# UBCMOCCA/mocca_envs

Measured on AMD Instinct MI355X. Metric: env-steps/sec, Walker3DCustomEnv-v0 @ 4096 envs, 1/2/4/8 MI355X, higher is better.
Workload: dtype f32; 1 GPU; Walker3DCustomEnv-v0, 4096 envs/GPU, flat ground, U(-1,1) action tape, auto-reset; max_rows=48, max_contacts=12, envs_per_gpu=4096, parallelism=independent env shards x1, no collective, preroll_steps=6096

## Files before the change

mocca_envs_amd/csrc/mocca_device.h:

```cpp
#pragma once

#include <hip/hip_runtime.h>
#include <stdint.h>

#include "mocca_model.h"
#include "mocca_philox.h"
#include "topo_walker3d.h"
#include "topo_cassie.h"
#include "topo_walker2d.h"
#include "topo_crab2d.h"
#include "topo_laikago.h"

#define DI __device__ __forceinline__

#ifndef MOCCA_NS
#define MOCCA_NS mocca
#endif
#ifndef MOCCA_MAXR
#define MOCCA_MAXR 48
#endif
#ifndef MOCCA_COMPACT
#define MOCCA_COMPACT 0
#endif

// ... 166 lines not shown
  unsigned long long* pace_acc;
  float* ep_ret;
  float* ep_masks;
  float* ep_bad;
  void* ep_rec;
  float* ep_totals;
  uint32_t ep_serial;
  float* robot_state;
  const float* base_value;
  int32_t* hf_field;
  int hf_stride, hf_n_fields, hf_redraw;
};
constexpr int ROBOT_STATE_STRIDE = 64;

DI void read_kernargs(StepArgs& la) {
  auto p = __builtin_amdgcn_kernarg_segment_ptr();
  asm volatile("" : "+s"(p));
  __builtin_memcpy(&la, p, sizeof(StepArgs));
}
template <bool LATE>
DI void late_args(StepArgs& la) {
  if constexpr (LATE) read_kernargs(la);
}
template <class T, int TASK, bool INJECT>
#ifdef MOCCA_NO_TRIM_7
constexpr bool LATE_ARGS = false;
#else
constexpr bool LATE_ARGS = INJECT || MAXR > 48 || !__is_base_of(TopoWalker3D, T) || (!COMPACT && TASK == MOCCA_TASK_WALKER3D_CUSTOM);
#endif

DI void wsync() {
  __builtin_amdgcn_fence(__ATOMIC_RELEASE, "wavefront");
  __builtin_amdgcn_wave_barrier();
  __builtin_amdgcn_fence(__ATOMIC_ACQUIRE, "wavefront");
}
DI float dot3(const float* a, const float* b) { return a[0] * b[0] + a[1] * b[1] + a[2] * b[2]; }
DI void cross3(const float* a, const float* b, float* o) {
  float x = a[1] * b[2] - a[2] * b[1], y = a[2] * b[0] - a[0] * b[2], z = a[0] * b[1] - a[1] * b[0];
  o[0] = x; o[1] = y; o[2] = z;
}
DI float dot6(const float* a, const float* b) {
  return a[0] * b[0] + a[1] * b[1] + a[2] * b[2] + a[3] * b[3] + a[4] * b[4] + a[5] * b[5];
}
DI void matvec3(const float* R, const float* x, float* o) {
  float a = R[0] * x[0] + R[1] * x[1] + R[2] * x[2];
  float b = R[3] * x[0] + R[4] * x[1] + R[5] * x[2];
// ... 489 lines not shown
        for (int k = 0; k < j; ++k) t -= own[k] * Afac[sym(j, k)];
        Afac[sym(j, j)] = readlane(rsq(t), j);
        own[j] = t * Afac[sym(j, j)];
#pragma unroll
        for (int i = j + 1; i < 6; ++i) Afac[sym(i, j)] = readlane(own[j], i);
      }
      chol6_solve(Afac, pA, a0);
    } else {
      float IA[21], pA[6];
#pragma unroll
      for (int i = 0; i < 6; ++i) {
        const float4 lo = *reinterpret_cast<const float4*>(L + L_B0 + 8 * i), hi = *reinterpret_cast<const float4*>(L + L_B0 + 8 * i + 4);
        const float rr_[6] = {lo.x, lo.y, lo.z, lo.w, hi.x, hi.y};
#pragma unroll
        for (int j = i; j < 6; ++j) IA[sym(i, j)] = rr_[j];
        pA[i] = hi.z;
      }
      float Ai[21];
      chol6_factor(IA, Ai);
      chol6_solve(Ai, pA, a0);
#pragma unroll
      for (int i = 0; i < 21; ++i) Afac[i] = unif(Ai[i]);
    }
#pragma unroll
    for (int i = 0; i < 6; ++i) abase[i] = -a0[i];
  }
  STAMP(11);
  {
    const int b = lane < T::NB ? lane : 0;
    float a[6], qdd = 0;
#pragma unroll
    for (int i = 0; i < 6; ++i) a[i] = abase[i];
#pragma unroll
    for (int k = 0; k < T::MAXD; ++k) {
      const int j = (int)((ppk >> (5 * k)) & 31ull);
      if (j != 0) {
        float U[6], S[6];
#pragma unroll
        for (int i = 0; i < 6; ++i) { a[i] += L[L_SV + SVS * j + SV_C + i]; U[i] = L[L_SV + SVS * j + SV_V + i]; S[i] = L[L_SV + SVS * j + i]; }
        qdd = L[L_SV + SVS * j + SV_UU] - dot6(U, a);
#pragma unroll
        for (int i = 0; i < 6; ++i) a[i] += S[i] * qdd;
      }
    }
    const float dt = M->dt;
    if (lane >= 1 && lane < T::NB) L[L_NU + 5 + b] = L[L_QD + b] + dt * qdd;
    if (lane == 0) {
      float om[3] = {L[L_BASE + 10], L[L_BASE + 11], L[L_BASE + 12]}, vl[3] = {L[L_BASE + 7], L[L_BASE + 8], L[L_BASE + 9]}, wxv[3];
      cross3(om, vl, wxv);
#pragma unroll
      for (int i = 0; i < 3; ++i) {
        L[L_NU + i] = om[i] + dt * a[i];
        L[L_NU + 3 + i] = vl[i] + dt * (a[3 + i] + wxv[i]);
      }
    }
    wsync();
  }
  STAMP(12);
}

DI void plane_space(const float* n, float* t1, float* t2) {
  if (fabsf(n[2]) > 0.70710678f) {
    const float a = n[1] * n[1] + n[2] * n[2], k = rsq(a);
    t1[0] = 0; t1[1] = -n[2] * k; t1[2] = n[1] * k;
    t2[0] = a * k; t2[1] = -n[0] * t1[2]; t2[2] = n[0] * t1[1];
  } else {
    const float a = n[0] * n[0] + n[1] * n[1], k = rsq(a);
    t1[0] = -n[1] * k; t1[1] = n[0] * k; t1[2] = 0;
    t2[0] = -n[2] * t1[1]; t2[1] = n[2] * t1[0]; t2[2] = a * k;
// ... 1808 lines not shown
```

mocca_envs_amd/csrc/mocca_kernels.h:

```cpp
#pragma once
#include <hip/hip_runtime.h>

#include "mocca.h"
#include "mocca_device.h"

namespace MOCCA_NS {

#ifndef MOCCA_WAVES_PER_EU
#define MOCCA_WAVES_PER_EU 4
#endif

DI void flush_obs(const float* L, float* dst, int lane, int obs_dim) {
#pragma unroll 1
  for (int k = lane; k < obs_dim; k += 64) dst[k] = L[L_OBS + k];
}
DI void keep_terminal_obs(const StepArgs& a, const float* L, int env, int lane) {
  wsync();
  if (a.final_obs) flush_obs(L, a.final_obs + (size_t)env * a.obs_dim, lane, a.obs_dim);
  wsync();
}

template <class T>
DI void keep_robot_state(const StepArgs& a, const float* L, int env, int lane) {
  static_assert(ROBOT_OBS<T> <= 64 && ROBOT_OBS<T> <= ROBOT_STATE_STRIDE, "one store per lane");
// ... 203 lines not shown
  cassie_observe(M, L, lane, cs, t.initz, jv, phase, obs);
  return {rew, 0};
}

template <class T, int TASK, bool INJECT = false>
__global__ __launch_bounds__(64, MOCCA_WAVES_PER_EU) void mocca_step_kernel(StepArgs a) {
  __shared__ float L[L_TOTAL];
  const int lane = threadIdx.x;
  if ((int)blockIdx.x >= a.n_envs) return;
  const int env = a.order ? uni(a.order[blockIdx.x]) : (int)blockIdx.x;
  ModelP M = (ModelP)a.model;
  float* st = a.dyn + (size_t)env * DYN_STRIDE;
  uint32_t* tk = a.task + (size_t)env * MOCCA_TASK_WORDS;
  float* ter = TASK == MOCCA_TASK_WALKER3D_STEPPER ? a.terrain + (size_t)env * TERRAIN_STRIDE : nullptr;
  float* obs_out = a.obs + (size_t)env * a.obs_dim;
  float* obs = L + L_OBS;
  int32_t* dbg = a.dbg ? a.dbg + (size_t)env * MOCCA_DEBUG_WORDS : nullptr;

  const bool warm_ld = INJECT || uni(__float_as_int(M->warmstart)) != 0, warm_st = warm_ld || a.persist_warm != 0;
  if (dbg && lane == 0) { dbg[16] = 0; dbg[17] = 0; dbg[18] = 0; }
  load_dyn(st, L, lane, T::NJ, T::NSLOT, warm_ld);
  pace_start(a, L, lane, INJECT ? 0 : a.pace);
  if (lane == 0) L[L_KEEPWARM] = __int_as_float((warm_st ? 1 : 0) | ((a.prio & PRIO_DELASSUS_VALU) ? 2 : 0));
  const unsigned long long ppk = T::path_packed(lane < T::NB ? lane : 0);
  ContactFlags fl = {0, 0, 0, 0, 0, 0, 0, 0, 0};
  int cover = 0;
  constexpr bool LATE = LATE_ARGS<T, TASK, INJECT>;
  StepArgs late, late_reset;
  const StepArgs& al = LATE ? late : a;
  if constexpr (TASK == MOCCA_TASK_CASSIE) {
    const int no = M->n_ordered, nctl = M->n_ctrl, mode = M->cassie_mode;
    float target = 0.0f;
    if (lane < nctl) {
      float base = M->ctrl_base[lane];
      if (mode != MOCCA_CASSIE_PLAIN) {
        const int f0 = traj_frame(a, M, (int)tk[MOCCA_TW_ISTEP]);
        base = (lane < nctl - 2 && M->residual_control) ? a.traj[(size_t)f0 * MOCCA_TRAJ_STRIDE + M->ctrl_oidx[lane]] : 0.0f;
      }
      target = base + (lane < nctl - 2 ? a.act[(size_t)env * (nctl - 2) + lane] : 0.0f);
    }
    if (lane < no) {
      L[L_JVEL + lane] = __uint_as_float(tk[MOCCA_TW_JVEL + lane]);
      L[L_Q0 + lane] = L[L_Q + M->ordered_body[lane]];
    }
    if (lane < MOCCA_MAX_BODIES) L[L_TAU + lane] = 0.0f;
    if (lane == 0) { L[L_Q] = 0.0f; L[L_QD] = 0.0f; }
    wsync();
// ... 212 lines not shown
```

mocca_envs_amd/csrc/topo_cassie.h:

```cpp
#pragma once
__device__ static const signed char kPathCassie[19][7] = {
  {-1, -1, -1, -1, -1, -1, -1},
  {1, -1, -1, -1, -1, -1, -1},
  {1, 2, -1, -1, -1, -1, -1},
  {1, 2, 3, -1, -1, -1, -1},
  {1, 2, 3, 4, -1, -1, -1},
  {1, 2, 3, 4, 5, -1, -1},
  {1, 2, 3, 4, 5, 6, -1},
  {1, 2, 3, 4, 5, 6, 7},
  {1, 2, 3, 8, -1, -1, -1},
  {1, 2, 3, 8, 9, -1, -1},
  {10, -1, -1, -1, -1, -1, -1},
  {10, 11, -1, -1, -1, -1, -1},
  {10, 11, 12, -1, -1, -1, -1},
  {10, 11, 12, 13, -1, -1, -1},
  {10, 11, 12, 13, 14, -1, -1},
  {10, 11, 12, 13, 14, 15, -1},
  {10, 11, 12, 13, 14, 15, 16},
  {10, 11, 12, 17, -1, -1, -1},
  {10, 11, 12, 17, 18, -1, -1},
};
__device__ static const signed char kChildCassie[19][2] = {
  {10, 1},
  {2, -1},
// ... 6 lines not shown
  {9, -1},
  {-1, -1},
  {11, -1},
  {12, -1},
  {17, 13},
  {14, -1},
  {15, -1},
  {16, -1},
  {-1, -1},
  {18, -1},
  {-1, -1},
};
__device__ static const signed char kLevelCassie[8][4] = {
  {-1, -1, -1, -1},
  {1, 10, -1, -1},
  {2, 11, -1, -1},
  {3, 12, -1, -1},
  {4, 13, 8, 17},
  {5, 14, 9, 18},
  {6, 15, -1, -1},
  {7, 16, -1, -1},
};
__device__ static const unsigned long long kPathPkCassie[19] = {0x0ull, 0x1ull, 0x41ull, 0xc41ull, 0x20c41ull, 0x520c41ull, 0xc520c41ull, 0x1cc520c41ull, 0x40c41ull, 0x940c41ull, 0xaull, 0x16aull, 0x316aull, 0x6b16aull, 0xe6b16aull, 0x1ee6b16aull, 0x41ee6b16aull, 0x8b16aull, 0x128b16aull};
struct TopoCassie {
  static constexpr int NB = 19;
  static constexpr int NJ = 18;
  static constexpr int ND = 24;
  static constexpr int MAXD = 7;
  static constexpr int MAXCH = 2;
  static constexpr int MAXW = 4;
  static constexpr int NG = 24;
  static constexpr int NSLOT = 24;
  static constexpr int NPAIR = 0;
  static constexpr int NCLOS = 2;
  static constexpr int NFEET = 2;
  static constexpr int parent(int b) { constexpr int t[19] = {-1, 0, 1, 2, 3, 4, 5, 6, 3, 8, 0, 10, 11, 12, 13, 14, 15, 12, 17}; return t[b]; }
  static constexpr int depth(int b) { constexpr int t[19] = {0, 1, 2, 3, 4, 5, 6, 7, 4, 5, 1, 2, 3, 4, 5, 6, 7, 4, 5}; return t[b]; }
  static constexpr unsigned anc_mask(int b) { constexpr unsigned t[19] = {0x0u, 0x2u, 0x6u, 0xeu, 0x1eu, 0x3eu, 0x7eu, 0xfeu, 0x10eu, 0x30eu, 0x400u, 0xc00u, 0x1c00u, 0x3c00u, 0x7c00u, 0xfc00u, 0x1fc00u, 0x21c00u, 0x61c00u}; return t[b]; }
  static __device__ __forceinline__ int path(int b, int k) { return kPathCassie[b][k]; }
  static __device__ __forceinline__ int child(int b, int k) { return kChildCassie[b][k]; }
  static __device__ __forceinline__ int level(int d, int s) { return kLevelCassie[d][s]; }
  static constexpr int clevel(int d, int s) { constexpr int t[8][4] = {{-1, -1, -1, -1}, {1, 10, -1, -1}, {2, 11, -1, -1}, {3, 12, -1, -1}, {4, 13, 8, 17}, {5, 14, 9, 18}, {6, 15, -1, -1}, {7, 16, -1, -1}}; return t[d][s]; }
  static constexpr bool massless(int b) { constexpr bool t[19] = {false, false, false, false, false, false, false, false, true, false, false, false, false, false, false, false, false, true, false}; return b >= 0 && t[b]; }
  static constexpr int ccarry(int b) { constexpr int t[19] = {-1, 2, 3, 4, 5, 6, 7, -1, 9, -1, 11, 12, 13, 14, 15, 16, -1, 18, -1}; return b < 0 ? -1 : t[b]; }
  static constexpr int cchild(int b, int k) { constexpr int t[19][2] = {{10, 1}, {2, -1}, {3, -1}, {8, 4}, {5, -1}, {6, -1}, {7, -1}, {-1, -1}, {9, -1}, {-1, -1}, {11, -1}, {12, -1}, {17, 13}, {14, -1}, {15, -1}, {16, -1}, {-1, -1}, {18, -1}, {-1, -1}}; return b < 0 ? -1 : t[b][k]; }
  static __device__ __forceinline__ unsigned long long path_packed(int b) { return kPathPkCassie[b]; }
};
```

mocca_envs_amd/csrc/topo_crab2d.h:

```cpp
#pragma once
__device__ static const signed char kPathCrab2D[7][3] = {
  {-1, -1, -1},
  {1, -1, -1},
  {1, 2, -1},
  {1, 2, 3},
  {4, -1, -1},
  {4, 5, -1},
  {4, 5, 6},
};
__device__ static const signed char kChildCrab2D[7][2] = {
  {4, 1},
  {2, -1},
  {3, -1},
  {-1, -1},
  {5, -1},
  {6, -1},
  {-1, -1},
};
__device__ static const signed char kLevelCrab2D[4][4] = {
  {-1, -1, -1, -1},
  {1, 4, -1, -1},
  {2, 5, -1, -1},
  {3, 6, -1, -1},
};
__device__ static const unsigned long long kPathPkCrab2D[7] = {0x0ull, 0x1ull, 0x41ull, 0xc41ull, 0x4ull, 0xa4ull, 0x18a4ull};
struct TopoCrab2D {
  static constexpr int NB = 7;
  static constexpr int NJ = 6;
  static constexpr int ND = 12;
  static constexpr int MAXD = 3;
  static constexpr int MAXCH = 2;
  static constexpr int MAXW = 4;
  static constexpr int NG = 7;
  static constexpr int NSLOT = 14;
  static constexpr int NPAIR = 9;
  static constexpr int NCLOS = 0;
  static constexpr int NFEET = 2;
  static constexpr int parent(int b) { constexpr int t[7] = {-1, 0, 1, 2, 0, 4, 5}; return t[b]; }
  static constexpr int depth(int b) { constexpr int t[7] = {0, 1, 2, 3, 1, 2, 3}; return t[b]; }
  static constexpr unsigned anc_mask(int b) { constexpr unsigned t[7] = {0x0u, 0x2u, 0x6u, 0xeu, 0x10u, 0x30u, 0x70u}; return t[b]; }
  static __device__ __forceinline__ int path(int b, int k) { return kPathCrab2D[b][k]; }
  static __device__ __forceinline__ int child(int b, int k) { return kChildCrab2D[b][k]; }
  static __device__ __forceinline__ int level(int d, int s) { return kLevelCrab2D[d][s]; }
  static constexpr int clevel(int d, int s) { constexpr int t[4][4] = {{-1, -1, -1, -1}, {1, 4, -1, -1}, {2, 5, -1, -1}, {3, 6, -1, -1}}; return t[d][s]; }
  static constexpr bool massless(int b) { constexpr bool t[7] = {false, false, false, false, false, false, false}; return b >= 0 && t[b]; }
  static constexpr int ccarry(int b) { constexpr int t[7] = {-1, 2, 3, -1, 5, 6, -1}; return b < 0 ? -1 : t[b]; }
  static constexpr int cchild(int b, int k) { constexpr int t[7][2] = {{4, 1}, {2, -1}, {3, -1}, {-1, -1}, {5, -1}, {6, -1}, {-1, -1}}; return b < 0 ? -1 : t[b][k]; }
  static __device__ __forceinline__ unsigned long long path_packed(int b) { return kPathPkCrab2D[b]; }
};
```

mocca_envs_amd/csrc/topo_laikago.h:

```cpp
#pragma once
__device__ static const signed char kPathLaikago[13][3] = {
  {-1, -1, -1},
  {1, -1, -1},
  {1, 2, -1},
  {1, 2, 3},
  {4, -1, -1},
  {4, 5, -1},
  {4, 5, 6},
  {7, -1, -1},
  {7, 8, -1},
  {7, 8, 9},
  {10, -1, -1},
  {10, 11, -1},
  {10, 11, 12},
};
__device__ static const signed char kChildLaikago[13][4] = {
  {10, 7, 4, 1},
  {2, -1, -1, -1},
  {3, -1, -1, -1},
  {-1, -1, -1, -1},
  {5, -1, -1, -1},
  {6, -1, -1, -1},
  {-1, -1, -1, -1},
  {8, -1, -1, -1},
  {9, -1, -1, -1},
  {-1, -1, -1, -1},
  {11, -1, -1, -1},
  {12, -1, -1, -1},
  {-1, -1, -1, -1},
};
__device__ static const signed char kLevelLaikago[4][4] = {
  {-1, -1, -1, -1},
  {1, 4, 7, 10},
  {2, 5, 8, 11},
  {3, 6, 9, 12},
};
__device__ static const unsigned long long kPathPkLaikago[13] = {0x0ull, 0x1ull, 0x41ull, 0xc41ull, 0x4ull, 0xa4ull, 0x18a4ull, 0x7ull, 0x107ull, 0x2507ull, 0xaull, 0x16aull, 0x316aull};
struct TopoLaikago {
  static constexpr int NB = 13;
  static constexpr int NJ = 12;
  static constexpr int ND = 18;
  static constexpr int MAXD = 3;
  static constexpr int MAXCH = 4;
  static constexpr int MAXW = 4;
  static constexpr int NG = 32;
  static constexpr int NSLOT = 32;
  static constexpr int NPAIR = 0;
  static constexpr int NCLOS = 0;
  static constexpr int NFEET = 4;
  static constexpr int parent(int b) { constexpr int t[13] = {-1, 0, 1, 2, 0, 4, 5, 0, 7, 8, 0, 10, 11}; return t[b]; }
  static constexpr int depth(int b) { constexpr int t[13] = {0, 1, 2, 3, 1, 2, 3, 1, 2, 3, 1, 2, 3}; return t[b]; }
  static constexpr unsigned anc_mask(int b) { constexpr unsigned t[13] = {0x0u, 0x2u, 0x6u, 0xeu, 0x10u, 0x30u, 0x70u, 0x80u, 0x180u, 0x380u, 0x400u, 0xc00u, 0x1c00u}; return t[b]; }
  static __device__ __forceinline__ int path(int b, int k) { return kPathLaikago[b][k]; }
  static __device__ __forceinline__ int child(int b, int k) { return kChildLaikago[b][k]; }
  static __device__ __forceinline__ int level(int d, int s) { return kLevelLaikago[d][s]; }
  static constexpr int clevel(int d, int s) { constexpr int t[4][4] = {{-1, -1, -1, -1}, {1, 4, 7, 10}, {2, 5, 8, 11}, {3, 6, 9, 12}}; return t[d][s]; }
  static constexpr bool massless(int b) { constexpr bool t[13] = {false, false, false, false, false, false, false, false, false, false, false, false, false}; return b >= 0 && t[b]; }
  static constexpr int ccarry(int b) { constexpr int t[13] = {-1, 2, 3, -1, 5, 6, -1, 8, 9, -1, 11, 12, -1}; return b < 0 ? -1 : t[b]; }
  static constexpr int cchild(int b, int k) { constexpr int t[13][4] = {{10, 7, 4, 1}, {2, -1, -1, -1}, {3, -1, -1, -1}, {-1, -1, -1, -1}, {5, -1, -1, -1}, {6, -1, -1, -1}, {-1, -1, -1, -1}, {8, -1, -1, -1}, {9, -1, -1, -1}, {-1, -1, -1, -1}, {11, -1, -1, -1}, {12, -1, -1, -1}, {-1, -1, -1, -1}}; return b < 0 ? -1 : t[b][k]; }
  static __device__ __forceinline__ unsigned long long path_packed(int b) { return kPathPkLaikago[b]; }
};
```

mocca_envs_amd/csrc/topo_walker2d.h:

```cpp
#pragma once
__device__ static const signed char kPathWalker2D[8][3] = {
  {-1, -1, -1},
  {1, -1, -1},
  {2, -1, -1},
  {2, 3, -1},
  {2, 3, 4},
  {5, -1, -1},
  {5, 6, -1},
  {5, 6, 7},
};
__device__ static const signed char kChildWalker2D[8][3] = {
  {5, 2, 1},
  {-1, -1, -1},
  {3, -1, -1},
  {4, -1, -1},
  {-1, -1, -1},
  {6, -1, -1},
  {7, -1, -1},
  {-1, -1, -1},
};
__device__ static const signed char kLevelWalker2D[4][4] = {
  {-1, -1, -1, -1},
  {2, 5, 1, -1},
  {3, 6, -1, -1},
  {4, 7, -1, -1},
};
__device__ static const unsigned long long kPathPkWalker2D[8] = {0x0ull, 0x1ull, 0x2ull, 0x62ull, 0x1062ull, 0x5ull, 0xc5ull, 0x1cc5ull};
struct TopoWalker2D {
  static constexpr int NB = 8;
  static constexpr int NJ = 7;
  static constexpr int ND = 13;
  static constexpr int MAXD = 3;
  static constexpr int MAXCH = 3;
  static constexpr int MAXW = 4;
  static constexpr int NG = 8;
  static constexpr int NSLOT = 15;
  static constexpr int NPAIR = 0;
  static constexpr int NCLOS = 0;
  static constexpr int NFEET = 2;
  static constexpr int parent(int b) { constexpr int t[8] = {-1, 0, 0, 2, 3, 0, 5, 6}; return t[b]; }
  static constexpr int depth(int b) { constexpr int t[8] = {0, 1, 1, 2, 3, 1, 2, 3}; return t[b]; }
  static constexpr unsigned anc_mask(int b) { constexpr unsigned t[8] = {0x0u, 0x2u, 0x4u, 0xcu, 0x1cu, 0x20u, 0x60u, 0xe0u}; return t[b]; }
  static __device__ __forceinline__ int path(int b, int k) { return kPathWalker2D[b][k]; }
  static __device__ __forceinline__ int child(int b, int k) { return kChildWalker2D[b][k]; }
  static __device__ __forceinline__ int level(int d, int s) { return kLevelWalker2D[d][s]; }
  static constexpr int clevel(int d, int s) { constexpr int t[4][4] = {{-1, -1, -1, -1}, {2, 5, 1, -1}, {3, 6, -1, -1}, {4, 7, -1, -1}}; return t[d][s]; }
  static constexpr bool massless(int b) { constexpr bool t[8] = {false, false, false, false, false, false, false, false}; return b >= 0 && t[b]; }
  static constexpr int ccarry(int b) { constexpr int t[8] = {-1, -1, 3, 4, -1, 6, 7, -1}; return b < 0 ? -1 : t[b]; }
  static constexpr int cchild(int b, int k) { constexpr int t[8][3] = {{5, 2, 1}, {-1, -1, -1}, {3, -1, -1}, {4, -1, -1}, {-1, -1, -1}, {6, -1, -1}, {7, -1, -1}, {-1, -1, -1}}; return b < 0 ? -1 : t[b][k]; }
  static __device__ __forceinline__ unsigned long long path_packed(int b) { return kPathPkWalker2D[b]; }
};
```

mocca_envs_amd/csrc/topo_walker3d.h:

```cpp
#pragma once
__device__ static const signed char kPathWalker3D[22][8] = {
  {-1, -1, -1, -1, -1, -1, -1, -1},
  {1, -1, -1, -1, -1, -1, -1, -1},
  {1, 2, -1, -1, -1, -1, -1, -1},
  {1, 2, 3, -1, -1, -1, -1, -1},
  {1, 2, 3, 4, -1, -1, -1, -1},
  {1, 2, 3, 4, 5, -1, -1, -1},
  {1, 2, 3, 4, 5, 6, -1, -1},
  {1, 2, 3, 4, 5, 6, 7, -1},
  {1, 2, 3, 4, 5, 6, 7, 8},
  {1, 2, 3, 9, -1, -1, -1, -1},
  {1, 2, 3, 9, 10, -1, -1, -1},
  {1, 2, 3, 9, 10, 11, -1, -1},
  {1, 2, 3, 9, 10, 11, 12, -1},
  {1, 2, 3, 9, 10, 11, 12, 13},
  {14, -1, -1, -1, -1, -1, -1, -1},
  {14, 15, -1, -1, -1, -1, -1, -1},
  {14, 15, 16, -1, -1, -1, -1, -1},
  {14, 15, 16, 17, -1, -1, -1, -1},
  {18, -1, -1, -1, -1, -1, -1, -1},
  {18, 19, -1, -1, -1, -1, -1, -1},
  {18, 19, 20, -1, -1, -1, -1, -1},
  {18, 19, 20, 21, -1, -1, -1, -1},
};
// ... 13 lines not shown
  {13, -1, -1},
  {-1, -1, -1},
  {15, -1, -1},
  {16, -1, -1},
  {17, -1, -1},
  {-1, -1, -1},
  {19, -1, -1},
  {20, -1, -1},
  {21, -1, -1},
  {-1, -1, -1},
};
__device__ static const signed char kLevelWalker3D[9][4] = {
  {-1, -1, -1, -1},
  {1, -1, 14, 18},
  {2, -1, 15, 19},
  {3, -1, 16, 20},
  {4, 9, 17, 21},
  {5, 10, -1, -1},
  {6, 11, -1, -1},
  {7, 12, -1, -1},
  {8, 13, -1, -1},
};
__device__ static const unsigned long long kPathPkWalker3D[22] = {0x0ull, 0x1ull, 0x41ull, 0xc41ull, 0x20c41ull, 0x520c41ull, 0xc520c41ull, 0x1cc520c41ull, 0x41cc520c41ull, 0x48c41ull, 0xa48c41ull, 0x16a48c41ull, 0x316a48c41ull, 0x6b16a48c41ull, 0xeull, 0x1eeull, 0x41eeull, 0x8c1eeull, 0x12ull, 0x272ull, 0x5272ull, 0xad272ull};
struct TopoWalker3D {
  static constexpr int NB = 22;
  static constexpr int NJ = 21;
  static constexpr int ND = 27;
  static constexpr int MAXD = 8;
  static constexpr int MAXCH = 3;
  static constexpr int MAXW = 4;
  static constexpr int NG = 22;
  static constexpr int NSLOT = 34;
  static constexpr int NPAIR = 141;
  static constexpr int NCLOS = 0;
  static constexpr int NFEET = 2;
  static constexpr int parent(int b) { constexpr int t[22] = {-1, 0, 1, 2, 3, 4, 5, 6, 7, 3, 9, 10, 11, 12, 0, 14, 15, 16, 0, 18, 19, 20}; return t[b]; }
  static constexpr int depth(int b) { constexpr int t[22] = {0, 1, 2, 3, 4, 5, 6, 7, 8, 4, 5, 6, 7, 8, 1, 2, 3, 4, 1, 2, 3, 4}; return t[b]; }
  static constexpr unsigned anc_mask(int b) { constexpr unsigned t[22] = {0x0u, 0x2u, 0x6u, 0xeu, 0x1eu, 0x3eu, 0x7eu, 0xfeu, 0x1feu, 0x20eu, 0x60eu, 0xe0eu, 0x1e0eu, 0x3e0eu, 0x4000u, 0xc000u, 0x1c000u, 0x3c000u, 0x40000u, 0xc0000u, 0x1c0000u, 0x3c0000u}; return t[b]; }
  static __device__ __forceinline__ int path(int b, int k) { return kPathWalker3D[b][k]; }
  static __device__ __forceinline__ int child(int b, int k) { return kChildWalker3D[b][k]; }
  static __device__ __forceinline__ int level(int d, int s) { return kLevelWalker3D[d][s]; }
  static constexpr int clevel(int d, int s) { constexpr int t[9][4] = {{-1, -1, -1, -1}, {1, -1, 14, 18}, {2, -1, 15, 19}, {3, -1, 16, 20}, {4, 9, 17, 21}, {5, 10, -1, -1}, {6, 11, -1, -1}, {7, 12, -1, -1}, {8, 13, -1, -1}}; return t[d][s]; }
  static constexpr bool massless(int b) { constexpr bool t[22] = {false, true, false, false, true, true, false, false, false, true, true, false, false, false, true, true, false, false, true, true, false, false}; return b >= 0 && t[b]; }
  static constexpr int ccarry(int b) { constexpr int t[22] = {-1, 2, 3, 4, 5, 6, 7, 8, -1, 10, 11, 12, 13, -1, 15, 16, 17, -1, 19, 20, 21, -1}; return b < 0 ? -1 : t[b]; }
  static constexpr int cchild(int b, int k) { constexpr int t[22][3] = {{18, 14, 1}, {2, -1, -1}, {3, -1, -1}, {9, 4, -1}, {5, -1, -1}, {6, -1, -1}, {7, -1, -1}, {8, -1, -1}, {-1, -1, -1}, {10, -1, -1}, {11, -1, -1}, {12, -1, -1}, {13, -1, -1}, {-1, -1, -1}, {15, -1, -1}, {16, -1, -1}, {17, -1, -1}, {-1, -1, -1}, {19, -1, -1}, {20, -1, -1}, {21, -1, -1}, {-1, -1, -1}}; return b < 0 ? -1 : t[b][k]; }
  static __device__ __forceinline__ unsigned long long path_packed(int b) { return kPathPkWalker3D[b]; }
};
```

mocca_envs_amd/model.py:

```python
from __future__ import annotations

import ctypes as C
import math
from dataclasses import dataclass, field
from types import SimpleNamespace
from typing import Dict, List, Optional, Sequence, Tuple

import numpy as np

MAX_BODIES = 24
MAX_GEOMS = 32
MAX_PAIRS = 192
MAX_FEET = 4
MAX_SLOTS = 40
MAGIC = 0x41434F4D
VERSION = 13

GEOM_SPHERE, GEOM_CAPSULE = 0, 1
TASK_WALKER3D_CUSTOM, TASK_WALKER3D_STEPPER, TASK_CASSIE, TASK_WALKER3D_PLANNER = 0, 1, 2, 3
TASK_WORDS = 40
TASK_RECORD = (
    ("WALK_TARGET_X", 0, 1, "f"), ("WALK_TARGET_Y", 1, 1, "f"), ("WALK_TARGET_Z", 2, 1, "f"),
    ("LINEAR_POTENTIAL", 3, 1, "f"), ("ANGULAR_POTENTIAL", 4, 1, "f"), ("CLOSE_COUNT", 5, 1, "i"), ("STOP_FRAMES", 6, 1, "f"),
    ("DONE", 7, 1, "i"), ("T", 8, 1, "i"), ("EPISODE", 9, 1, "i"), ("DRAW", 10, 1, "i"), ("MIRRORED", 11, 1, "i"),
# ... 959 lines not shown
    for b in range(1, m.n_bodies):
        m.gain[b] = 40.0
        m.init_q[b] = -math.pi / 6 if links[b].name.endswith("lower_leg_2_upper_leg_joint") else 0.0
    m.dt, m.n_substeps = (1.0 / 240.0, 4) if stepper else (1.0 / 480.0, 8)
    _put(m.init_pos, (0.25, 0.0, 0.53) if stepper else (0.0, 0.0, 0.56))
    m.init_quat[3] = 1.0
    _set_walker_task(m, termination_height=0.0)
    _set_mirror(m, [0, 1, 2, 6, 7, 8], [3, 4, 5, 9, 10, 11])
    m.task_flags |= TASKF_BODY_CONTACT
    if stepper:
        _put(m.init_vel, (0.5, 0.0, 0.25))
        set_stepper_params(m, quadruped=True, plank_class=plank_class)
        m.task_flags = (m.task_flags & ~TASKF_BODY_CONTACT) | TASKF_QUADRUPED_STEPPER
    return m.finalize_tables()


def joint_limits(m: MoccaModel) -> Tuple[np.ndarray, np.ndarray]:
    nj = m.n_joints
    lo = np.array([m.jlo[b] for b in range(1, nj + 1)], dtype=np.float32)
    hi = np.array([m.jhi[b] for b in range(1, nj + 1)], dtype=np.float32)
    return lo, hi


def topology_header(m: MoccaModel, name: str = "Walker3D") -> str:
    nb = m.n_bodies
    parent = [m.parent[b] for b in range(nb)]
    depth = [m.depth[b] for b in range(nb)]
    maxd = max(depth)
    children = [[c for c in range(nb) if parent[c] == b] for b in range(nb)]
    maxc = max(len(c) for c in children)
    by_depth = [[b for b in range(nb) if depth[b] == d] for d in range(maxd + 1)]
    maxw = max(4, max(len(l) for l in by_depth[1:]))
    slot_of, carry = {}, [-1] * nb
    levels = [[-1] * maxw for _ in range(maxd + 1)]
    for d in range(maxd, 0, -1):
        taken = set()
        for b in by_depth[d]:
            for c in sorted(children[b]):
                if slot_of[c] not in taken:
                    slot_of[b], carry[b] = slot_of[c], c
                    taken.add(slot_of[c])
                    break
        for b in by_depth[d]:
            if b not in slot_of:
                slot_of[b] = min(set(range(maxw)) - taken)
                taken.add(slot_of[b])
        for b in by_depth[d]:
            levels[d][slot_of[b]] = b
    path = []
    for b in range(nb):
        p, cur = [], b
        while cur > 0:
            p.append(cur)
            cur = parent[cur]
        p = p[::-1]
        path.append(p + [-1] * (maxd - len(p)))

    def arr(vals):
        return "{" + ", ".join(str(v) for v in vals) + "}"

    lines = [
        "// GENERATED by mocca_envs_amd.model.topology_header() -- do not edit.",
        "// Kinematic tree of %s as compile-time tables (numbers live in the MoccaModel blob)." % name,
        "#pragma once",
        "// runtime-indexed copies (per-lane lookups)",
        "__device__ static const signed char kPath%s[%d][%d] = {" % (name, nb, maxd),
    ]
    lines += ["  %s," % arr(p) for p in path]
    lines += ["};", "__device__ static const signed char kChild%s[%d][%d] = {" % (name, nb, maxc)]
    lines += ["  %s," % arr(sorted(c, reverse=True) + [-1] * (maxc - len(c))) for c in children]
    lines += ["};", "__device__ static const signed char kLevel%s[%d][%d] = {" % (name, maxd + 1, maxw)]
    lines += ["  %s," % arr(l) for l in levels]
    lines += [
        "};",
        "__device__ static const unsigned long long kPathPk%s[%d] = %s;" % (
            name, nb, arr(["0x%xull" % sum(((path[b][k] if path[b][k] >= 0 else 0) << (5 * k)) for k in range(maxd)) for b in range(nb)])),
        "struct Topo%s {" % name,
        "  static constexpr int NB = %d;        // bodies incl. floating base" % nb,
        "  static constexpr int NJ = %d;        // hinges" % (nb - 1),
        "  static constexpr int ND = %d;        // generalised velocities" % (nb + 5),
        "  static constexpr int MAXD = %d;      // tree depth" % maxd,
        "  static constexpr int MAXCH = %d;     // children per body" % maxc,
        "  static constexpr int MAXW = %d;      // bodies per level" % maxw,
        "  static constexpr int NG = %d;        // geoms" % m.n_geoms,
        "  static constexpr int NSLOT = %d;     // terrain contact slots" % m.n_slots,
        "  static constexpr int NPAIR = %d;     // self-collision candidate pairs" % m.n_pairs,
        "  static constexpr int NCLOS = %d;     // point-to-point loop closures" % m.n_closures,
        "  static constexpr int NFEET = %d;     // feet (entries of the observation, robots.py:74-86)" % m.n_feet,
        "  // constexpr functions (implicitly __host__ __device__ under hipcc) fold after unrolling",
        "  static constexpr int parent(int b) { constexpr int t[%d] = %s; return t[b]; }" % (nb, arr(parent)),
        "  static constexpr int depth(int b) { constexpr int t[%d] = %s; return t[b]; }" % (nb, arr(depth)),
        "  static constexpr unsigned anc_mask(int b) { constexpr unsigned t[%d] = %s; return t[b]; }"
        % (nb, arr(["0x%xu" % m.anc_mask[b] for b in range(nb)])),
        "  static __device__ __forceinline__ int path(int b, int k) { return kPath%s[b][k]; }" % name,
        "  static __device__ __forceinline__ int child(int b, int k) { return kChild%s[b][k]; }" % name,
        "  static __device__ __forceinline__ int level(int d, int s) { return kLevel%s[d][s]; }" % name,
        "  // compile-time versions: with the loops over k / d unrolled these cost a few VALU ops and NO memory access",
        "  // (a dependent global table load per tree level / path step is what dominated the latency-bound phases)",
        "  static constexpr int clevel(int d, int s) { constexpr int t[%d][%d] = {%s}; return t[d][s]; }"
        % (maxd + 1, maxw, ", ".join(arr(l) for l in levels)),
        "  // links without mass or inertia (the intermediate links of multi-hinge joints): a tree level that holds only such links skips the",
        "  // reads of its (all-zero) link inertia and bias force in the ABA inward pass; mocca_create() checks the blob against this table",
        "  static constexpr bool massless(int b) { constexpr bool t[%d] = %s; return b >= 0 && t[b]; }"
        % (nb, arr(["true" if (m.mass[b] == 0.0 and all(m.inertia[b][i] == 0.0 for i in range(6)) and b > 0) else "false" for b in range(nb)])),
        "  // the child whose articulated inertia stays in registers (same slot, next level), -1 if none",
        "  static constexpr int ccarry(int b) { constexpr int t[%d] = %s; return b < 0 ? -1 : t[b]; }" % (nb, arr(carry)),
        "  static constexpr int cchild(int b, int k) { constexpr int t[%d][%d] = {%s}; return b < 0 ? -1 : t[b][k]; }"
        % (nb, maxc, ", ".join(arr(sorted(c, reverse=True) + [-1] * (maxc - len(c))) for c in children)),
        "  // the lane's own root->body path, 5 bits per step (0 = past the end: joints are numbered from 1): loaded once per kernel, two VGPRs, then",
        "  // every path step is a v_bfe -- no table access inside the walks",
        "  static __device__ __forceinline__ unsigned long long path_packed(int b) { return kPathPk%s[b]; }" % name,
        "};",
        "",
    ]
    return "\n".join(lines)


def write_topology_headers(outdir: Optional[str] = None) -> None:
    import os
    outdir = outdir or os.path.join(os.path.dirname(os.path.abspath(__file__)), "csrc")
    with open(os.path.join(outdir, "topo_walker3d.h"), "w") as f:
        f.write(topology_header(compile_walker3d(), "Walker3D"))
    with open(os.path.join(outdir, "topo_cassie.h"), "w") as f:
        f.write(topology_header(compile_cassie(), "Cassie"))
    with open(os.path.join(outdir, "topo_walker2d.h"), "w") as f:
        f.write(topology_header(compile_walker2d(), "Walker2D"))
    with open(os.path.join(outdir, "topo_crab2d.h"), "w") as f:
        f.write(topology_header(compile_crab2d(), "Crab2D"))
    with open(os.path.join(outdir, "topo_laikago.h"), "w") as f:
        f.write(topology_header(compile_laikago(), "Laikago"))


if __name__ == "__main__":
    write_topology_headers()
# ... 1 lines not shown
```

Measured before the change: 43.04 million env-steps/s.

## Run ABA outward pass level-by-level with chains laid out across DPP rows

```diff
diff --git a/mocca_envs_amd/csrc/mocca_device.h b/mocca_envs_amd/csrc/mocca_device.h
--- a/mocca_envs_amd/csrc/mocca_device.h
+++ b/mocca_envs_amd/csrc/mocca_device.h
@@ -212,6 +212,12 @@
 DI void late_args(StepArgs& la) {
   if constexpr (LATE) read_kernargs(la);
 }
+template <class T>
+#ifdef MOCCA_NO_TRIM_8
+constexpr bool OUTWARD_ROUNDS = false;
+#else
+constexpr bool OUTWARD_ROUNDS = T::OUTWARD_DPP && !COMPACT;
+#endif
 template <class T, int TASK, bool INJECT>
 #ifdef MOCCA_NO_TRIM_7
 constexpr bool LATE_ARGS = false;
@@ -747,29 +753,67 @@
 #pragma unroll
       for (int i = 0; i < 21; ++i) Afac[i] = unif(Ai[i]);
     }
+    if constexpr (OUTWARD_ROUNDS<T>) {
+#pragma unroll
+      for (int i = 0; i < 6; ++i) pin1(a0[i]);
+    }
 #pragma unroll
     for (int i = 0; i < 6; ++i) abase[i] = -a0[i];
   }
   STAMP(11);
   {
-    const int b = lane < T::NB ? lane : 0;
     float a[6], qdd = 0;
+    int b;
+    bool store;
 #pragma unroll
     for (int i = 0; i < 6; ++i) a[i] = abase[i];
-#pragma unroll
-    for (int k = 0; k < T::MAXD; ++k) {
-      const int j = (int)((ppk >> (5 * k)) & 31ull);
-      if (j != 0) {
-        float U[6], S[6];
-#pragma unroll
-        for (int i = 0; i < 6; ++i) { a[i] += L[L_SV + SVS * j + SV_C + i]; U[i] = L[L_SV + SVS * j + SV_V + i]; S[i] = L[L_SV + SVS * j + i]; }
-        qdd = L[L_SV + SVS * j + SV_UU] - dot6(U, a);
-#pragma unroll
-        for (int i = 0; i < 6; ++i) a[i] += S[i] * qdd;
+    if constexpr (OUTWARD_ROUNDS<T>) {
+      const int ol = T::out_lane(ppk);
+      b = ol & 31;
+      store = (unsigned)(ol - 1) < 31u;
+      static_assert(SV_V == 6 && SV_C == 12 && SV_UU == 18 && SVS % 4 == 0 && L_SV % 4 == 0, "the body record as five 16-byte reads");
+      const float4* rec = reinterpret_cast<const float4*>(L + L_SV + SVS * b);
+      const float4 r0 = rec[0], r1 = rec[1], r2 = rec[2], r3 = rec[3], r4 = rec[4];
+      const float S[6] = {r0.x, r0.y, r0.z, r0.w, r1.x, r1.y}, V[6] = {r1.z, r1.w, r2.x, r2.y, r2.z, r2.w};
+      const float c[6] = {r3.x, r3.y, r3.z, r3.w, r4.x, r4.y}, uu = r4.z;
+      float t[6], ab[6];
+#pragma unroll
+      for (int i = 0; i < 6; ++i) { pin1(a[i]); asm("v_add_f32_e32 %0, %1, %2" : "=v"(t[i]) : "v"(a[i]), "v"(c[i])); }
+#pragma unroll
+      for (int k = 0; k < T::MAXD; ++k) {
+        if (k > 0) {
+          asm("s_nop 1\n\t"
+              "v_add_f32_dpp %0, %6, %12 row_shr:1 row_mask:0xf bank_mask:0xf\n\t"
+              "v_add_f32_dpp %1, %7, %13 row_shr:1 row_mask:0xf bank_mask:0xf\n\t"
+              "v_add_f32_dpp %2, %8, %14 row_shr:1 row_mask:0xf bank_mask:0xf\n\t"
+              "v_add_f32_dpp %3, %9, %15 row_shr:1 row_mask:0xf bank_mask:0xf\n\t"
+              "v_add_f32_dpp %4, %10, %16 row_shr:1 row_mask:0xf bank_mask:0xf\n\t"
+              "v_add_f32_dpp %5, %11, %17 row_shr:1 row_mask:0xf bank_mask:0xf"
+              : "+v"(t[0]), "+v"(t[1]), "+v"(t[2]), "+v"(t[3]), "+v"(t[4]), "+v"(t[5])
+              : "v"(ab[0]), "v"(ab[1]), "v"(ab[2]), "v"(ab[3]), "v"(ab[4]), "v"(ab[5]), "v"(c[0]), "v"(c[1]), "v"(c[2]), "v"(c[3]), "v"(c[4]), "v"(c[5]));
+        }
+        qdd = uu - dot6(V, t);
+#pragma unroll
+        for (int i = 0; i < 6; ++i) ab[i] = t[i] + S[i] * qdd;
       }
+    } else {
+      b = lane < T::NB ? lane : 0;
+      store = lane >= 1 && lane < T::NB;
+#pragma unroll
+      for (int k = 0; k < T::MAXD; ++k) {
+        const int j = (int)((ppk >> (5 * k)) & 31ull);
+        if (j != 0) {
+          float U[6], S[6];
+#pragma unroll
+          for (int i = 0; i < 6; ++i) { a[i] += L[L_SV + SVS * j + SV_C + i]; U[i] = L[L_SV + SVS * j + SV_V + i]; S[i] = L[L_SV + SVS * j + i]; }
+          qdd = L[L_SV + SVS * j + SV_UU] - dot6(U, a);
+#pragma unroll
+          for (int i = 0; i < 6; ++i) a[i] += S[i] * qdd;
+        }
+      }
     }
     const float dt = M->dt;
-    if (lane >= 1 && lane < T::NB) L[L_NU + 5 + b] = L[L_QD + b] + dt * qdd;
+    if (store) L[L_NU + 5 + b] = L[L_QD + b] + dt * qdd;
     if (lane == 0) {
       float om[3] = {L[L_BASE + 10], L[L_BASE + 11], L[L_BASE + 12]}, vl[3] = {L[L_BASE + 7], L[L_BASE + 8], L[L_BASE + 9]}, wxv[3];
       cross3(om, vl, wxv);
diff --git a/mocca_envs_amd/csrc/mocca_kernels.h b/mocca_envs_amd/csrc/mocca_kernels.h
--- a/mocca_envs_amd/csrc/mocca_kernels.h
+++ b/mocca_envs_amd/csrc/mocca_kernels.h
@@ -249,7 +249,7 @@
   load_dyn(st, L, lane, T::NJ, T::NSLOT, warm_ld);
   pace_start(a, L, lane, INJECT ? 0 : a.pace);
   if (lane == 0) L[L_KEEPWARM] = __int_as_float((warm_st ? 1 : 0) | ((a.prio & PRIO_DELASSUS_VALU) ? 2 : 0));
-  const unsigned long long ppk = T::path_packed(lane < T::NB ? lane : 0);
+  const unsigned long long ppk = OUTWARD_ROUNDS<T> ? T::lane_packed(lane) : T::path_packed(lane < T::NB ? lane : 0);
   ContactFlags fl = {0, 0, 0, 0, 0, 0, 0, 0, 0};
   int cover = 0;
   constexpr bool LATE = LATE_ARGS<T, TASK, INJECT>;
diff --git a/mocca_envs_amd/csrc/topo_cassie.h b/mocca_envs_amd/csrc/topo_cassie.h
--- a/mocca_envs_amd/csrc/topo_cassie.h
+++ b/mocca_envs_amd/csrc/topo_cassie.h
@@ -52,6 +52,7 @@
   {7, 16, -1, -1},
 };
 __device__ static const unsigned long long kPathPkCassie[19] = {0x0ull, 0x1ull, 0x41ull, 0xc41ull, 0x20c41ull, 0x520c41ull, 0xc520c41ull, 0x1cc520c41ull, 0x40c41ull, 0x940c41ull, 0xaull, 0x16aull, 0x316aull, 0x6b16aull, 0xe6b16aull, 0x1ee6b16aull, 0x41ee6b16aull, 0x8b16aull, 0x128b16aull};
+__device__ static const unsigned long long kLanePkCassie[64] = {0x400000000000000ull, 0x800000000000001ull, 0xc00000000000041ull, 0x1000000000000c41ull, 0x1400000000020c41ull, 0x1800000000520c41ull, 0x1c0000000c520c41ull, 0x1cc520c41ull, 0x40c41ull, 0x940c41ull, 0xaull, 0x16aull, 0x316aull, 0x6b16aull, 0xe6b16aull, 0x1ee6b16aull, 0x840000041ee6b16aull, 0x880000000008b16aull, 0x8c0000000128b16aull, 0x2000000000000000ull, 0x2400000000000000ull, 0x0ull, 0x0ull, 0x0ull, 0x0ull, 0x0ull, 0x0ull, 0x0ull, 0x0ull, 0x0ull, 0x0ull, 0x0ull, 0x2800000000000000ull, 0x2c00000000000000ull, 0x3000000000000000ull, 0x3400000000000000ull, 0x3800000000000000ull, 0x3c00000000000000ull, 0x4000000000000000ull, 0x0ull, 0x0ull, 0x0ull, 0x0ull, 0x0ull, 0x0ull, 0x0ull, 0x0ull, 0x0ull, 0xa800000000000000ull, 0xac00000000000000ull, 0xb000000000000000ull, 0x4400000000000000ull, 0x4800000000000000ull, 0x0ull, 0x0ull, 0x0ull, 0x0ull, 0x0ull, 0x0ull, 0x0ull, 0x0ull, 0x0ull, 0x0ull, 0x0ull};
 struct TopoCassie {
   static constexpr int NB = 19;
   static constexpr int NJ = 18;
@@ -75,4 +76,9 @@
   static constexpr int ccarry(int b) { constexpr int t[19] = {-1, 2, 3, 4, 5, 6, 7, -1, 9, -1, 11, 12, 13, 14, 15, 16, -1, 18, -1}; return b < 0 ? -1 : t[b]; }
   static constexpr int cchild(int b, int k) { constexpr int t[19][2] = {{10, 1}, {2, -1}, {3, -1}, {8, 4}, {5, -1}, {6, -1}, {7, -1}, {-1, -1}, {9, -1}, {-1, -1}, {11, -1}, {12, -1}, {17, 13}, {14, -1}, {15, -1}, {16, -1}, {-1, -1}, {18, -1}, {-1, -1}}; return b < 0 ? -1 : t[b][k]; }
   static __device__ __forceinline__ unsigned long long path_packed(int b) { return kPathPkCassie[b]; }
+  static constexpr bool OUTWARD_DPP = false;
+  static constexpr int out_body(int lane) { constexpr int t[64] = {1, 2, 3, 4, 5, 6, 7, -1, -1, -1, -1, -1, -1, -1, -1, -1, 1, 2, 3, 8, 9, -1, -1, -1, -1, -1, -1, -1, -1, -1, -1, -1, 10, 11, 12, 13, 14, 15, 16, -1, -1, -1, -1, -1, -1, -1, -1, -1, 10, 11, 12, 17, 18, -1, -1, -1, -1, -1, -1, -1, -1, -1, -1, -1}; return t[lane]; }
+  static constexpr bool out_primary(int lane) { constexpr bool t[64] = {true, true, true, true, true, true, true, false, false, false, false, false, false, false, false, false, false, false, false, true, true, false, false, false, false, false, false, false, false, false, false, false, true, true, true, true, true, true, true, false, false, false, false, false, false, false, false, false, false, false, false, true, true, false, false, false, false, false, false, false, false, false, false, false}; return t[lane]; }
+  static __device__ __forceinline__ unsigned long long lane_packed(int lane) { return kLanePkCassie[lane]; }
+  static __device__ __forceinline__ int out_lane(unsigned long long lane_pk) { return (int)(lane_pk >> 58); }
 };
diff --git a/mocca_envs_amd/csrc/topo_crab2d.h b/mocca_envs_amd/csrc/topo_crab2d.h
--- a/mocca_envs_amd/csrc/topo_crab2d.h
+++ b/mocca_envs_amd/csrc/topo_crab2d.h
@@ -24,6 +24,7 @@
   {3, 6, -1, -1},
 };
 __device__ static const unsigned long long kPathPkCrab2D[7] = {0x0ull, 0x1ull, 0x41ull, 0xc41ull, 0x4ull, 0xa4ull, 0x18a4ull};
+__device__ static const unsigned long long kLanePkCrab2D[64] = {0x400000000000000ull, 0x800000000000001ull, 0xc00000000000041ull, 0xc41ull, 0x4ull, 0xa4ull, 0x18a4ull, 0x0ull, 0x0ull, 0x0ull, 0x0ull, 0x0ull, 0x0ull, 0x0ull, 0x0ull, 0x0ull, 0x1000000000000000ull, 0x1400000000000000ull, 0x1800000000000000ull, 0x0ull, 0x0ull, 0x0ull, 0x0ull, 0x0ull, 0x0ull, 0x0ull, 0x0ull, 0x0ull, 0x0ull, 0x0ull, 0x0ull, 0x0ull, 0x0ull, 0x0ull, 0x0ull, 0x0ull, 0x0ull, 0x0ull, 0x0ull, 0x0ull, 0x0ull, 0x0ull, 0x0ull, 0x0ull, 0x0ull, 0x0ull, 0x0ull, 0x0ull, 0x0ull, 0x0ull, 0x0ull, 0x0ull, 0x0ull, 0x0ull, 0x0ull, 0x0ull, 0x0ull, 0x0ull, 0x0ull, 0x0ull, 0x0ull, 0x0ull, 0x0ull, 0x0ull};
 struct TopoCrab2D {
   static constexpr int NB = 7;
   static constexpr int NJ = 6;
@@ -47,4 +48,9 @@
   static constexpr int ccarry(int b) { constexpr int t[7] = {-1, 2, 3, -1, 5, 6, -1}; return b < 0 ? -1 : t[b]; }
   static constexpr int cchild(int b, int k) { constexpr int t[7][2] = {{4, 1}, {2, -1}, {3, -1}, {-1, -1}, {5, -1}, {6, -1}, {-1, -1}}; return b < 0 ? -1 : t[b][k]; }
   static __device__ __forceinline__ unsigned long long path_packed(int b) { return kPathPkCrab2D[b]; }
+  static constexpr bool OUTWARD_DPP = true;
+  static constexpr int out_body(int lane) { constexpr int t[64] = {1, 2, 3, -1, -1, -1, -1, -1, -1, -1, -1, -1, -1, -1, -1, -1, 4, 5, 6, -1, -1, -1, -1, -1, -1, -1, -1, -1, -1, -1, -1, -1, -1, -1, -1, -1, -1, -1, -1, -1, -1, -1, -1, -1, -1, -1, -1, -1, -1, -1, -1, -1, -1, -1, -1, -1, -1, -1, -1, -1, -1, -1, -1, -1}; return t[lane]; }
+  static constexpr bool out_primary(int lane) { constexpr bool t[64] = {true, true, true, false, false, false, false, false, false, false, false, false, false, false, false, false, true, true, true, false, false, false, false, false, false, false, false, false, false, false, false, false, false, false, false, false, false, false, false, false, false, false, false, false, false, false, false, false, false, false, false, false, false, false, false, false, false, false, false, false, false, false, false, false}; return t[lane]; }
+  static __device__ __forceinline__ unsigned long long lane_packed(int lane) { return kLanePkCrab2D[lane]; }
+  static __device__ __forceinline__ int out_lane(unsigned long long lane_pk) { return (int)(lane_pk >> 58); }
 };
diff --git a/mocca_envs_amd/csrc/topo_laikago.h b/mocca_envs_amd/csrc/topo_laikago.h
--- a/mocca_envs_amd/csrc/topo_laikago.h
+++ b/mocca_envs_amd/csrc/topo_laikago.h
@@ -36,6 +36,7 @@
   {3, 6, 9, 12},
 };
 __device__ static const unsigned long long kPathPkLaikago[13] = {0x0ull, 0x1ull, 0x41ull, 0xc41ull, 0x4ull, 0xa4ull, 0x18a4ull, 0x7ull, 0x107ull, 0x2507ull, 0xaull, 0x16aull, 0x316aull};
+__device__ static const unsigned long long kLanePkLaikago[64] = {0x400000000000000ull, 0x800000000000001ull, 0xc00000000000041ull, 0xc41ull, 0x4ull, 0xa4ull, 0x18a4ull, 0x7ull, 0x107ull, 0x2507ull, 0xaull, 0x16aull, 0x316aull, 0x0ull, 0x0ull, 0x0ull, 0x1000000000000000ull, 0x1400000000000000ull, 0x1800000000000000ull, 0x0ull, 0x0ull, 0x0ull, 0x0ull, 0x0ull, 0x0ull, 0x0ull, 0x0ull, 0x0ull, 0x0ull, 0x0ull, 0x0ull, 0x0ull, 0x1c00000000000000ull, 0x2000000000000000ull, 0x2400000000000000ull, 0x0ull, 0x0ull, 0x0ull, 0x0ull, 0x0ull, 0x0ull, 0x0ull, 0x0ull, 0x0ull, 0x0ull, 0x0ull, 0x0ull, 0x0ull, 0x2800000000000000ull, 0x2c00000000000000ull, 0x3000000000000000ull, 0x0ull, 0x0ull, 0x0ull, 0x0ull, 0x0ull, 0x0ull, 0x0ull, 0x0ull, 0x0ull, 0x0ull, 0x0ull, 0x0ull, 0x0ull};
 struct TopoLaikago {
   static constexpr int NB = 13;
   static constexpr int NJ = 12;
@@ -59,4 +60,9 @@
   static constexpr int ccarry(int b) { constexpr int t[13] = {-1, 2, 3, -1, 5, 6, -1, 8, 9, -1, 11, 12, -1}; return b < 0 ? -1 : t[b]; }
   static constexpr int cchild(int b, int k) { constexpr int t[13][4] = {{10, 7, 4, 1}, {2, -1, -1, -1}, {3, -1, -1, -1}, {-1, -1, -1, -1}, {5, -1, -1, -1}, {6, -1, -1, -1}, {-1, -1, -1, -1}, {8, -1, -1, -1}, {9, -1, -1, -1}, {-1, -1, -1, -1}, {11, -1, -1, -1}, {12, -1, -1, -1}, {-1, -1, -1, -1}}; return b < 0 ? -1 : t[b][k]; }
   static __device__ __forceinline__ unsigned long long path_packed(int b) { return kPathPkLaikago[b]; }
+  static constexpr bool OUTWARD_DPP = true;
+  static constexpr int out_body(int lane) { constexpr int t[64] = {1, 2, 3, -1, -1, -1, -1, -1, -1, -1, -1, -1, -1, -1, -1, -1, 4, 5, 6, -1, -1, -1, -1, -1, -1, -1, -1, -1, -1, -1, -1, -1, 7, 8, 9, -1, -1, -1, -1, -1, -1, -1, -1, -1, -1, -1, -1, -1, 10, 11, 12, -1, -1, -1, -1, -1, -1, -1, -1, -1, -1, -1, -1, -1}; return t[lane]; }
+  static constexpr bool out_primary(int lane) { constexpr bool t[64] = {true, true, true, false, false, false, false, false, false, false, false, false, false, false, false, false, true, true, true, false, false, false, false, false, false, false, false, false, false, false, false, false, true, true, true, false, false, false, false, false, false, false, false, false, false, false, false, false, true, true, true, false, false, false, false, false, false, false, false, false, false, false, false, false}; return t[lane]; }
+  static __device__ __forceinline__ unsigned long long lane_packed(int lane) { return kLanePkLaikago[lane]; }
+  static __device__ __forceinline__ int out_lane(unsigned long long lane_pk) { return (int)(lane_pk >> 58); }
 };
diff --git a/mocca_envs_amd/csrc/topo_walker2d.h b/mocca_envs_amd/csrc/topo_walker2d.h
--- a/mocca_envs_amd/csrc/topo_walker2d.h
+++ b/mocca_envs_amd/csrc/topo_walker2d.h
@@ -26,6 +26,7 @@
   {4, 7, -1, -1},
 };
 __device__ static const unsigned long long kPathPkWalker2D[8] = {0x0ull, 0x1ull, 0x2ull, 0x62ull, 0x1062ull, 0x5ull, 0xc5ull, 0x1cc5ull};
+__device__ static const unsigned long long kLanePkWalker2D[64] = {0x400000000000000ull, 0x1ull, 0x2ull, 0x62ull, 0x1062ull, 0x5ull, 0xc5ull, 0x1cc5ull, 0x0ull, 0x0ull, 0x0ull, 0x0ull, 0x0ull, 0x0ull, 0x0ull, 0x0ull, 0x800000000000000ull, 0xc00000000000000ull, 0x1000000000000000ull, 0x0ull, 0x0ull, 0x0ull, 0x0ull, 0x0ull, 0x0ull, 0x0ull, 0x0ull, 0x0ull, 0x0ull, 0x0ull, 0x0ull, 0x0ull, 0x1400000000000000ull, 0x1800000000000000ull, 0x1c00000000000000ull, 0x0ull, 0x0ull, 0x0ull, 0x0ull, 0x0ull, 0x0ull, 0x0ull, 0x0ull, 0x0ull, 0x0ull, 0x0ull, 0x0ull, 0x0ull, 0x0ull, 0x0ull, 0x0ull, 0x0ull, 0x0ull, 0x0ull, 0x0ull, 0x0ull, 0x0ull, 0x0ull, 0x0ull, 0x0ull, 0x0ull, 0x0ull, 0x0ull, 0x0ull};
 struct TopoWalker2D {
   static constexpr int NB = 8;
   static constexpr int NJ = 7;
@@ -49,4 +50,9 @@
   static constexpr int ccarry(int b) { constexpr int t[8] = {-1, -1, 3, 4, -1, 6, 7, -1}; return b < 0 ? -1 : t[b]; }
   static constexpr int cchild(int b, int k) { constexpr int t[8][3] = {{5, 2, 1}, {-1, -1, -1}, {3, -1, -1}, {4, -1, -1}, {-1, -1, -1}, {6, -1, -1}, {7, -1, -1}, {-1, -1, -1}}; return b < 0 ? -1 : t[b][k]; }
   static __device__ __forceinline__ unsigned long long path_packed(int b) { return kPathPkWalker2D[b]; }
+  static constexpr bool OUTWARD_DPP = true;
+  static constexpr int out_body(int lane) { constexpr int t[64] = {1, -1, -1, -1, -1, -1, -1, -1, -1, -1, -1, -1, -1, -1, -1, -1, 2, 3, 4, -1, -1, -1, -1, -1, -1, -1, -1, -1, -1, -1, -1, -1, 5, 6, 7, -1, -1, -1, -1, -1, -1, -1, -1, -1, -1, -1, -1, -1, -1, -1, -1, -1, -1, -1, -1, -1, -1, -1, -1, -1, -1, -1, -1, -1}; return t[lane]; }
+  static constexpr bool out_primary(int lane) { constexpr bool t[64] = {true, false, false, false, false, false, false, false, false, false, false, false, false, false, false, false, true, true, true, false, false, false, false, false, false, false, false, false, false, false, false, false, true, true, true, false, false, false, false, false, false, false, false, false, false, false, false, false, false, false, false, false, false, false, false, false, false, false, false, false, false, false, false, false}; return t[lane]; }
+  static __device__ __forceinline__ unsigned long long lane_packed(int lane) { return kLanePkWalker2D[lane]; }
+  static __device__ __forceinline__ int out_lane(unsigned long long lane_pk) { return (int)(lane_pk >> 58); }
 };
diff --git a/mocca_envs_amd/csrc/topo_walker3d.h b/mocca_envs_amd/csrc/topo_walker3d.h
--- a/mocca_envs_amd/csrc/topo_walker3d.h
+++ b/mocca_envs_amd/csrc/topo_walker3d.h
@@ -59,6 +59,7 @@
   {8, 13, -1, -1},
 };
 __device__ static const unsigned long long kPathPkWalker3D[22] = {0x0ull, 0x1ull, 0x41ull, 0xc41ull, 0x20c41ull, 0x520c41ull, 0xc520c41ull, 0x1cc520c41ull, 0x41cc520c41ull, 0x48c41ull, 0xa48c41ull, 0x16a48c41ull, 0x316a48c41ull, 0x6b16a48c41ull, 0xeull, 0x1eeull, 0x41eeull, 0x8c1eeull, 0x12ull, 0x272ull, 0x5272ull, 0xad272ull};
+__device__ static const unsigned long long kLanePkWalker3D[64] = {0x400000000000000ull, 0x800000000000001ull, 0xc00000000000041ull, 0x1000000000000c41ull, 0x1400000000020c41ull, 0x1800000000520c41ull, 0x1c0000000c520c41ull, 0x20000001cc520c41ull, 0x41cc520c41ull, 0x48c41ull, 0xa48c41ull, 0x16a48c41ull, 0x316a48c41ull, 0x6b16a48c41ull, 0xeull, 0x1eeull, 0x84000000000041eeull, 0x880000000008c1eeull, 0x8c00000000000012ull, 0x2400000000000272ull, 0x2800000000005272ull, 0x2c000000000ad272ull, 0x3000000000000000ull, 0x3400000000000000ull, 0x0ull, 0x0ull, 0x0ull, 0x0ull, 0x0ull, 0x0ull, 0x0ull, 0x0ull, 0x3800000000000000ull, 0x3c00000000000000ull, 0x4000000000000000ull, 0x4400000000000000ull, 0x0ull, 0x0ull, 0x0ull, 0x0ull, 0x0ull, 0x0ull, 0x0ull, 0x0ull, 0x0ull, 0x0ull, 0x0ull, 0x0ull, 0x4800000000000000ull, 0x4c00000000000000ull, 0x5000000000000000ull, 0x5400000000000000ull, 0x0ull, 0x0ull, 0x0ull, 0x0ull, 0x0ull, 0x0ull, 0x0ull, 0x0ull, 0x0ull, 0x0ull, 0x0ull, 0x0ull};
 struct TopoWalker3D {
   static constexpr int NB = 22;
   static constexpr int NJ = 21;
@@ -82,4 +83,9 @@
   static constexpr int ccarry(int b) { constexpr int t[22] = {-1, 2, 3, 4, 5, 6, 7, 8, -1, 10, 11, 12, 13, -1, 15, 16, 17, -1, 19, 20, 21, -1}; return b < 0 ? -1 : t[b]; }
   static constexpr int cchild(int b, int k) { constexpr int t[22][3] = {{18, 14, 1}, {2, -1, -1}, {3, -1, -1}, {9, 4, -1}, {5, -1, -1}, {6, -1, -1}, {7, -1, -1}, {8, -1, -1}, {-1, -1, -1}, {10, -1, -1}, {11, -1, -1}, {12, -1, -1}, {13, -1, -1}, {-1, -1, -1}, {15, -1, -1}, {16, -1, -1}, {17, -1, -1}, {-1, -1, -1}, {19, -1, -1}, {20, -1, -1}, {21, -1, -1}, {-1, -1, -1}}; return b < 0 ? -1 : t[b][k]; }
   static __device__ __forceinline__ unsigned long long path_packed(int b) { return kPathPkWalker3D[b]; }
+  static constexpr bool OUTWARD_DPP = true;
+  static constexpr int out_body(int lane) { constexpr int t[64] = {1, 2, 3, 4, 5, 6, 7, 8, -1, -1, -1, -1, -1, -1, -1, -1, 1, 2, 3, 9, 10, 11, 12, 13, -1, -1, -1, -1, -1, -1, -1, -1, 14, 15, 16, 17, -1, -1, -1, -1, -1, -1, -1, -1, -1, -1, -1, -1, 18, 19, 20, 21, -1, -1, -1, -1, -1, -1, -1, -1, -1, -1, -1, -1}; return t[lane]; }
+  static constexpr bool out_primary(int lane) { constexpr bool t[64] = {true, true, true, true, true, true, true, true, false, false, false, false, false, false, false, false, false, false, false, true, true, true, true, true, false, false, false, false, false, false, false, false, true, true, true, true, false, false, false, false, false, false, false, false, false, false, false, false, true, true, true, true, false, false, false, false, false, false, false, false, false, false, false, false}; return t[lane]; }
+  static __device__ __forceinline__ unsigned long long lane_packed(int lane) { return kLanePkWalker3D[lane]; }
+  static __device__ __forceinline__ int out_lane(unsigned long long lane_pk) { return (int)(lane_pk >> 58); }
 };
diff --git a/mocca_envs_amd/model.py b/mocca_envs_amd/model.py
--- a/mocca_envs_amd/model.py
+++ b/mocca_envs_amd/model.py
@@ -1005,6 +1005,27 @@
     return lo, hi
 
 
+OUTWARD_ROWS, OUTWARD_ROW_LANES = 4, 16
+OUTWARD_SHIFT = 58
+
+
+def outward_layout(parent: List[int], n_closures: int = 0) -> Tuple[bool, List[int]]:
+    nb = len(parent)
+    lanes = [-1] * (OUTWARD_ROWS * OUTWARD_ROW_LANES)
+    chains = []
+    for leaf in (b for b in range(1, nb) if b not in parent[1:]):
+        c, cur = [], leaf
+        while cur > 0:
+            c.append(cur)
+            cur = parent[cur]
+        chains.append(c[::-1])
+    if len(chains) > OUTWARD_ROWS or any(len(c) > OUTWARD_ROW_LANES for c in chains):
+        return False, lanes
+    for r, c in enumerate(chains):
+        lanes[OUTWARD_ROW_LANES * r:OUTWARD_ROW_LANES * r + len(c)] = c
+    return n_closures == 0, lanes
+
+
 def topology_header(m: MoccaModel, name: str = "Walker3D") -> str:
     nb = m.n_bodies
     parent = [m.parent[b] for b in range(nb)]
@@ -1038,6 +1059,11 @@
             cur = parent[cur]
         p = p[::-1]
         path.append(p + [-1] * (maxd - len(p)))
+    outward_dpp, out_lanes = outward_layout(parent, m.n_closures)
+    out_primary = [b >= 0 and out_lanes.index(b) == l for l, b in enumerate(out_lanes)]
+    out_lane_bits = [0 if b < 0 else b + (0 if p else 32) for b, p in zip(out_lanes, out_primary)]
+    pathpk = [sum(((path[b][k] if path[b][k] >= 0 else 0) << (5 * k)) for k in range(maxd)) for b in range(nb)]
+    assert 5 * maxd <= OUTWARD_SHIFT and nb <= 32, "the packed path and the outward pass's lane bits share one 64-bit word"
 
     def arr(vals):
         return "{" + ", ".join(str(v) for v in vals) + "}"
@@ -1057,7 +1083,11 @@
     lines += [
         "};",
         "__device__ static const unsigned long long kPathPk%s[%d] = %s;" % (
-            name, nb, arr(["0x%xull" % sum(((path[b][k] if path[b][k] >= 0 else 0) << (5 * k)) for k in range(maxd)) for b in range(nb)])),
+            name, nb, arr(["0x%xull" % v for v in pathpk])),
+        "// per LANE: the packed path of the lane's body in the lane = body layout (kPathPk of body `lane`, 0 behind the last body) and, in the top six",
+        "// bits, the lane's body in the level-by-level ABA outward pass (model.py outward_layout): + 32 on a lane that repeats a shared trunk, 0 idle",
+        "__device__ static const unsigned long long kLanePk%s[%d] = %s;" % (
+            name, len(out_lanes), arr(["0x%xull" % ((pathpk[l] if l < nb else 0) | (ol << OUTWARD_SHIFT)) for l, ol in enumerate(out_lane_bits)])),
         "struct Topo%s {" % name,
         "  static constexpr int NB = %d;        // bodies incl. floating base" % nb,
         "  static constexpr int NJ = %d;        // hinges" % (nb - 1),
@@ -1093,6 +1123,16 @@
         "  // the lane's own root->body path, 5 bits per step (0 = past the end: joints are numbered from 1): loaded once per kernel, two VGPRs, then",
         "  // every path step is a v_bfe -- no table access inside the walks",
         "  static __device__ __forceinline__ unsigned long long path_packed(int b) { return kPathPk%s[b]; }" % name,
+        "  // ABA outward pass, level by level: every root->leaf chain on consecutive lanes from the start of a 16-lane DPP row, so a body's parent is",
+        "  // the lane to its left (model.py outward_layout).  out_body: the lane's body, -1 idle; out_primary: the one lane of a body that stores",
+        "  // (a trunk that chains share is repeated in their rows); OUTWARD_DPP: at most four chains of at most 16 bodies and no loop closures",
+        "  static constexpr bool OUTWARD_DPP = %s;" % ("true" if outward_dpp else "false"),
+        "  static constexpr int out_body(int lane) { constexpr int t[%d] = %s; return t[lane]; }" % (len(out_lanes), arr(out_lanes)),
+        "  static constexpr bool out_primary(int lane) { constexpr bool t[%d] = %s; return t[lane]; }"
+        % (len(out_lanes), arr(["true" if p else "false" for p in out_primary])),
+        "  // what the step kernel keeps per lane across the substeps: path_packed of body `lane` (0 behind the last body), out_lane above it",
+        "  static __device__ __forceinline__ unsigned long long lane_packed(int lane) { return kLanePk%s[lane]; }" % name,
+        "  static __device__ __forceinline__ int out_lane(unsigned long long lane_pk) { return (int)(lane_pk >> %d); }" % OUTWARD_SHIFT,
         "};",
         "",
     ]
```

After: 44.31 million env-steps/s (median of 6 runs). 1.03x the previous value.
